# ltronchin/LatentAugment

Measured on AMD Instinct MI355X. Metric: augmented images/sec (256^2, 20 latent steps), higher is better.
Workload: dtype f32 (scaled split-fp16x2 on fp16 MFMA, fp32 accumulate); 1 GPU; SG2 config-f 256x256 2-ch, random-init G, batch=8/GPU, 20 latent steps; global_batch=8, parallelism=dp1

## Files before the change

### latentaugment_amd/csrc/la_conv_bf16.hip

```cpp
#include "la_conv_device.h"
#include <atomic>
#include <type_traits>

typedef __bf16 bf16x8 __attribute__((ext_vector_type(8)));
typedef _Float16 f16x8 __attribute__((ext_vector_type(8)));

#define FMT_BF16X3 3
#define FMT_BF16X2 2
#define FMT_F16X2 16
#define PRESPLIT_HDR 512

template <bool F16>
__device__ __forceinline__ f32x16 la_mma(bf16x8 a, bf16x8 b, f32x16 c) {
    if constexpr (F16) return __builtin_amdgcn_mfma_f32_32x32x16_f16(__builtin_bit_cast(f16x8, a), __builtin_bit_cast(f16x8, b), c, 0, 0, 0);
    else return __builtin_amdgcn_mfma_f32_32x32x16_bf16(a, b, c, 0, 0, 0);
}

#define KCB 32

__host__ __device__ static inline int pack_mp(int M) { return (M + 31) & ~31; }
__device__ __forceinline__ long pack_slab_offset(int m, int k) {
    return ((((long)(m >> 5) * 2 + (k >> 4)) * 64 + ((k >> 3) & 1) * 32 + (m & 31)) << 3) + (k & 7);
}
__global__ void la_pack_bf16_kernel(const float* __restrict__ w, __bf16* __restrict__ out, int cout, int cin, int ktaps,
// ... 241 lines not shown
__global__ __launch_bounds__(256) void la_presplit_t_kernel(const float* __restrict__ in, long in_bstride,
                                                           const float* __restrict__ scale, int scale_stride,
                                                           const float* __restrict__ xscale, int xs_fan, unsigned* __restrict__ out, int C, long HW,
                                                           LaInMask mk) {
    constexpr int EW = F16 ? 1 : 2;
    __shared__ unsigned tile[EW][64][33];
    const int cc = blockIdx.y, b = blockIdx.z, nck = gridDim.y;
    const long p0 = (long)blockIdx.x * 64;
    if (mk.p_hi > 0 && (p0 + 64 <= mk.p_lo || p0 >= mk.p_hi)) return;
    const float xs = F16 ? la_xs_get(xscale, b, xs_fan) : 1.f;
    {
        const int px = threadIdx.x & 63, cg = threadIdx.x >> 6;
        const long p = p0 + px;
#pragma unroll
        for (int i = 0; i < 8; ++i) {
            const int cl = cg * 8 + i, c = cc * KCB + cl;
            float v = 0.f;
            if (c < C && p < HW) {
                const long o = (long)b * in_bstride + (long)c * HW + p;
                v = in[o] * ((scale ? scale[(long)b * scale_stride + c] : 1.f) * xs);
                if (mk.y) v *= la_act_bwd_from_y(mk.y[o], mk.act, mk.alpha, mk.gain, mk.clamp);
                v *= mk.in_gain;
            }
            if (F16) {
                const _Float16 h = (_Float16)v;
                const _Float16 l = (_Float16)(v - (float)h);
                tile[0][px][cl] = (unsigned)__builtin_bit_cast(unsigned short, h) | ((unsigned)__builtin_bit_cast(unsigned short, l) << 16);
            } else {
                unsigned short t[3];
#pragma unroll
                for (int q = 0; q < 3; ++q) {
                    const __bf16 h = (__bf16)v;
                    t[q] = __builtin_bit_cast(unsigned short, h);
                    v -= (float)h;
                }
                tile[0][px][cl] = (unsigned)t[0] | ((unsigned)t[1] << 16);
                tile[EW - 1][px][cl] = (unsigned)t[2];
            }
        }
    }
    __syncthreads();
    {
        const int px = threadIdx.x >> 2, qt = threadIdx.x & 3;
        const long p = p0 + px;
        if (p < HW) {
            unsigned* op = out + (((long)b * nck + cc) * HW + p) * (KCB * EW) + qt * 8 * EW;
            if (F16) {
                unsigned e[8];
#pragma unroll
                for (int k = 0; k < 8; ++k) e[k] = tile[0][px][qt * 8 + k];
                uint4* rec = reinterpret_cast<uint4*>(out + (((long)b * nck + cc) * HW + p) * KCB);
                rec[qt] = make_uint4(__builtin_amdgcn_perm(e[1], e[0], 0x05040100u), __builtin_amdgcn_perm(e[3], e[2], 0x05040100u),
                                     __builtin_amdgcn_perm(e[5], e[4], 0x05040100u), __builtin_amdgcn_perm(e[7], e[6], 0x05040100u));
                rec[4 + qt] = make_uint4(__builtin_amdgcn_perm(e[1], e[0], 0x07060302u), __builtin_amdgcn_perm(e[3], e[2], 0x07060302u),
                                         __builtin_amdgcn_perm(e[5], e[4], 0x07060302u), __builtin_amdgcn_perm(e[7], e[6], 0x07060302u));
            } else {
#pragma unroll
                for (int k = 0; k < 4; ++k)
                    reinterpret_cast<uint4*>(op)[k] = make_uint4(tile[0][px][qt * 8 + 2 * k], tile[EW - 1][px][qt * 8 + 2 * k],
                                                                 tile[0][px][qt * 8 + 2 * k + 1], tile[EW - 1][px][qt * 8 + 2 * k + 1]);
            }
        }
    }
}

static inline size_t presplit_hdr_bytes(int B, int C) { return (PRESPLIT_HDR + (size_t)B * C * PM_NS * 4 + 255) & ~(size_t)255; }
size_t la_conv_presplit_bytes(int B, int C, int Hin, int Win) {
    return (size_t)B * la_cdiv(C, KCB) * KCB * Hin * Win * 8 + 16 + presplit_hdr_bytes(B, C);
}

static int prepare_scale(LaConvArgs& a, hipStream_t stream) {
    if (a.precision != LA_PREC_F16X2 || a.acc_scale_x) return LA_OK;
    const long HW = (long)a.Hin * a.Win;
    const size_t hb = presplit_hdr_bytes(a.B, a.C);
    LA_CHECK_ARG(a.ws && a.ws_bytes >= hb, "conv: split precisions need a workspace (la_modconv_workspace_bytes)");
    LA_CHECK_ARG(((size_t)a.ws & 15) == 0, "conv: workspace must be 16-byte aligned");
    LA_CHECK_ARG(a.B <= 64, "conv: split precisions support at most 64 samples per launch");
    char* base = static_cast<char*>(a.ws);
    float* xscale = reinterpret_cast<float*>(base);
    float* pm = reinterpret_cast<float*>(base + PRESPLIT_HDR);
    int ns = (int)(HW / 8192);
    ns = ns < 1 ? 1 : (ns > PM_NS ? PM_NS : ns);
    if (a.in_pmax) {
        hipLaunchKernelGGL(la_xscale_pmax_kernel, dim3(a.B), dim3(1024), 0, stream, a.in_pmax, a.in_pmax_nseg > 0 ? a.in_pmax_nseg : 1, a.in_scale,
                           a.scale_stride, xscale, a.C, 1.f);
    } else {
        hipLaunchKernelGGL(la_plane_absmax_kernel, dim3(ns, a.C, a.B), dim3(256), 0, stream, a.in, a.in_bstride, a.in_scale,
                           a.scale_stride, pm, a.C, HW, ns);
        hipLaunchKernelGGL(la_xscale_kernel, dim3(a.B), dim3(256), 0, stream, pm, xscale, a.C * ns);
    }
    LA_CHECK_LAUNCH();
    a.acc_scale_x = xscale; a.acc_scale_fan = 1;
    a.ws = base + hb;
    a.ws_bytes -= hb;
    return LA_OK;
}

bool la_conv_bf16_uses_halo(const LaConvArgs& a) {
    if (a.precision == LA_PREC_F32 || a.in_q) return false;
    if (a.in_mask_y || (a.in_gain != 0.f && a.in_gain != 1.f)) return false;
    if (a.in_sy != 1 || a.in_sx != 1 || a.out_sy != 1 || a.out_sx != 1 || a.out_oy != 0 || a.out_ox != 0) return false;
    if ((a.Gx & 31) != 0 || (a.Gy & 3) != 0 || a.Gy != a.Hout || a.Gx != a.Wout || a.ntaps != 9) return false;
    if ((long)a.Gy * a.Gx < (la_dev_knob(LA_KNOB_HALO_MING) ? la_dev_knob(LA_KNOB_HALO_MING) : 1157)) return false;
    if ((long)a.C * a.Hin * a.Win >= (1l << 28) || a.C > 4096) return false;
    for (int t = 0; t < a.ntaps; ++t)
        if (a.tap_dy[t] < -1 || a.tap_dy[t] > 1 || a.tap_dx[t] < -1 || a.tap_dx[t] > 1) return false;
    return true;
}

int la_conv_prepare_input(LaConvArgs& a, hipStream_t stream) {
    if (a.precision == LA_PREC_F32 || a.in_q) return LA_OK;
    const long HW = (long)a.Hin * a.Win;
    struct Bracket { int slot; hipStream_t st; ~Bracket() { la_prof_close(slot, st); } };
    if (la_conv_bf16_uses_halo(a)) {
        if (a.precision != LA_PREC_F16X2 || a.acc_scale_x) return LA_OK;
        Bracket br{la_prof_open(LA_PC_PRESPLIT, 0.0, a.in_pmax ? 0.0 : 4.0 * a.B * (double)a.C * HW * (a.in_bstride ? 1.0 : 1.0 / a.B), stream), stream};
        return prepare_scale(a, stream);
    }
    Bracket br{la_prof_open(LA_PC_PRESPLIT, 0.0, 4.0 * a.B * (double)a.C * HW * ((a.in_bstride ? 1.0 : 1.0 / a.B) + 1.0), stream), stream};
    const size_t qb = la_conv_presplit_bytes(a.B, a.C, a.Hin, a.Win);
    LA_CHECK_ARG(a.ws && a.ws_bytes >= qb, "conv: split precisions need a workspace (la_modconv_workspace_bytes)");
    LA_CHECK_ARG(((size_t)a.ws & 15) == 0, "conv: workspace must be 16-byte aligned");
    LA_CHECK_ARG(a.B <= 64, "conv: split precisions support at most 64 samples per launch");
    LA_CHECK_ARG(qb < 0x7ff00000u, "conv: pre-split operand too large for 32-bit buffer offsets");
    char* base = static_cast<char*>(a.ws);
    const size_t ws_bytes = a.ws_bytes;
    const dim3 pgrid((unsigned)la_cdiv(HW, 64), (unsigned)la_cdiv(a.C, KCB), (unsigned)a.B);
    const LaInMask mk{a.in_mask_y, a.in_mask_act, a.in_mask_alpha, a.in_mask_gain, a.in_mask_clamp, a.in_gain != 0.f ? a.in_gain : 1.f,
                      a.in_row_hi > 0 ? (long)a.in_row_lo * a.Win : 0, a.in_row_hi > 0 ? (long)a.in_row_hi * a.Win : 0};
    LA_CHECK_ARG((!a.in_mask_y && mk.in_gain == 1.f) || a.acc_scale_x || a.precision != LA_PREC_F16X2, "conv: an input mask needs a preset operand scale");
    if (a.precision == LA_PREC_F16X2) {
        int rc = prepare_scale(a, stream);
        if (rc) return rc;
        void* q = a.ws;
        hipLaunchKernelGGL(la_presplit_t_kernel<true>, pgrid, dim3(256), 0, stream, a.in, a.in_bstride, a.in_scale, a.scale_stride,
                           a.acc_scale_x, a.acc_scale_fan, (unsigned*)q, a.C, HW, mk);
        a.in_q = q;
    } else {
        void* q = base + presplit_hdr_bytes(a.B, a.C);
        hipLaunchKernelGGL(la_presplit_t_kernel<false>, pgrid, dim3(256), 0, stream, a.in, a.in_bstride, a.in_scale, a.scale_stride,
                           (const float*)nullptr, 0, (unsigned*)q, a.C, HW, mk);
        a.in_q = q;
    }
    LA_CHECK_LAUNCH();
    const size_t off = (qb + 255) & ~(size_t)255;
    a.ws = ws_bytes > off ? base + off : nullptr;
    a.ws_bytes = ws_bytes > off ? ws_bytes - off : 0;
    return LA_OK;
}

typedef unsigned int u32x4 __attribute__((ext_vector_type(4)));
typedef unsigned int u32x2 __attribute__((ext_vector_type(2)));
#define BPITCH 64
template <int MT, bool SPLIT, int FMT, int WV, int MF = 0>
__global__ __launch_bounds__(256) __attribute__((amdgpu_waves_per_eu(WV))) void la_conv_bf16_kernel(LaConvArgs a_in) {
    static_assert(MF == 0 ? WV == 2 : (MF <= 2 && WV == 3 && FMT == FMT_F16X2 && MT == 128),
                  "the 16x16x32 forms exist for the three-wave fp16 x2 kernel on 128-row tiles, the 32x32x16 form for two waves");
    LaConvArgs a = a_in;
    int bz = blockIdx.z;
    int bx = blockIdx.x;
    if (a_in.nphase > 0) {
        int ph;
        if (SPLIT) {
            ph = 0;
#pragma unroll
            for (int q = 1; q < LA_CONV_MAX_PHASES; ++q)
                if (q < a_in.nphase && bx >= a_in.ph[q].tile0) ph = q;
            bx -= a_in.ph[ph].tile0;
            a.splitk_ws = a_in.splitk_ws + a_in.ph[ph].ws_off;
        } else {
            ph = bz / a_in.B;
            bz -= ph * a_in.B;
        }
        a.Gy = a_in.ph[ph].Gy; a.Gx = a_in.ph[ph].Gx; a.out_oy = a_in.ph[ph].out_oy; a.out_ox = a_in.ph[ph].out_ox; a.ntaps = a_in.ph[ph].ntaps;
#pragma unroll
        for (int t = 0; t < LA_CONV_PHASE_TAPS; ++t) { a.tap_dy[t] = a_in.ph[ph].tap_dy[t]; a.tap_dx[t] = a_in.ph[ph].tap_dx[t]; a.tap_w[t] = a_in.ph[ph].tap_w[t]; }
    }
    constexpr int NTERM = FMT == FMT_BF16X3 ? 3 : 2;
    constexpr bool F16 = FMT == FMT_F16X2;
    constexpr int WM_ = MT == 128 ? 4 : 2;
    constexpr int WN_ = 4 / WM_;
    constexpr int TM = 1;
    constexpr int NJ = 4 / WN_;
    constexpr int EB = F16 ? 4 : 8;
    constexpr int BPLANE = NT * BPITCH;
    constexpr int BBUF = NTERM * BPLANE;
    extern __shared__ __attribute__((aligned(16))) unsigned char smem[];
    float (*red)[MT] = reinterpret_cast<float (*)[MT]>(smem);

    const int tid = threadIdx.x;
    const int lane = tid & 63, wid = tid >> 6;
    const int wm = wid / WN_, wn = wid % WN_;
    int ntile = bx;
    const int m0 = blockIdx.y * MT;
    const int G = a.Gy * a.Gx;
    const int Ntot = SPLIT ? a.B * G : G;
    if (!SPLIT) {
        int t0 = 0, nt = (int)gridDim.x;
        if (a.row_hi > 0) {
            const int tall = (G + NT - 1) / NT;
            t0 = (a.row_lo * a.Gx) / NT;
            int t1 = ((a.row_hi < a.Gy ? a.row_hi : a.Gy) * a.Gx + NT - 1) / NT;
            t1 = t1 < tall ? t1 : tall;
            nt = t1 - t0;
            for (int j = (int)blockIdx.x; j < tall - nt; j += (int)gridDim.x) la_conv_zero_partials<MT>(a, bz, m0, j < t0 ? j : j + nt);
            const int n8 = (int)gridDim.x;
            if ((n8 & 7) == 0) ntile = (blockIdx.x & 7) * (n8 >> 3) + (blockIdx.x >> 3);
            if (ntile >= nt) return;
        } else if ((nt & 7) == 0) ntile = (blockIdx.x & 7) * (nt >> 3) + (blockIdx.x >> 3);
        ntile += t0;
    }
    if (!SPLIT && (long)ntile * NT >= G) return;
    const int l31 = lane & 31, lh = lane >> 5;

    const int n_l = tid & (NT - 1);
    const int khalf = tid >> 7;
    const int nidx_l = ntile * NT + n_l;
    const bool nvalid = nidx_l < Ntot;
    const int b_l = SPLIT ? (nvalid ? nidx_l / G : 0) : bz;
    const int g_l = SPLIT ? nidx_l - b_l * G : nidx_l;
    const int gy_l = nvalid ? g_l / a.Gx : 0;
    const int gx_l = nvalid ? g_l - gy_l * a.Gx : 0;
    const int iy0 = gy_l * a.in_sy, ix0 = gx_l * a.in_sx;
    const unsigned HWin = (unsigned)(a.Hin * a.Win);
    const int vy0 = a.in_row_hi > 0 ? a.in_row_lo : 0, vy1 = a.in_row_hi > 0 ? a.in_row_hi : a.Hin;
    constexpr bool PIECES = FMT == FMT_F16X2;
    constexpr unsigned OOB = 0x7ff00000u;
    unsigned plin[4] = {0u, 0u, 0u, 0u}, pinv[4] = {0u, 0u, 0u, 0u};
    if constexpr (PIECES) {
#pragma unroll
        for (int k = 0; k < 4; ++k) {
            const int n_k = k * 32 + (tid >> 3);
            const int nidx = ntile * NT + n_k;
            const bool pv = nidx < Ntot;
            const int bb = SPLIT ? (pv ? nidx / G : 0) : bz;
            const int g = SPLIT ? nidx - bb * G : nidx;
            const int gy = pv ? g / a.Gx : 0, gx = pv ? g - gy * a.Gx : 0;
            const int py = gy * a.in_sy, px = gx * a.in_sx;
            const unsigned base = (SPLIT ? (unsigned)bb * ((unsigned)((a.C + KCB - 1) / KCB) * KCB * HWin * 4u) : 0u) + (unsigned)(tid & 7) * 16u;
            plin[k] = base + (unsigned)(py * a.Win + px) * (unsigned)(KCB * EB);
            unsigned m = 0u;
#pragma unroll
            for (int t = 0; t < LA_CONV_MAX_TAPS; ++t) {
                const int iy = py + a.tap_dy[t], ix = px + a.tap_dx[t];
                const bool bad = !pv || iy < vy0 || iy >= vy1 || ix < 0 || ix >= a.Win;
                m |= (bad ? 1u : 0u) << t;
            }
            pinv[k] = m;
        }
    }

    const int nck = (a.C + KCB - 1) / KCB;
    int ck_beg = 0, ck_end = nck;
    if (SPLIT) {
        const int per = (nck + a.ksplit - 1) / a.ksplit;
        ck_beg = blockIdx.z * per;
        ck_end = ck_beg + per < nck ? ck_beg + per : nck;
    }
    const int ntaps = a.ntaps;
    const int nstep = ck_end > ck_beg ? (ck_end - ck_beg) * ntaps : 0;
    const long term_elems = a.wgt_bf16_term_elems;
    const unsigned samp_bytes = (unsigned)nck * KCB * HWin * EB;
    const auto rs_in = __builtin_amdgcn_make_buffer_rsrc(
        const_cast<char*>(static_cast<const char*>(a.in_q)) + (SPLIT ? (size_t)0 : (size_t)bz * samp_bytes), 0,
        (int)(SPLIT ? samp_bytes * (unsigned)a.B : samp_bytes), 0x00020000);
    const auto rs_w = __builtin_amdgcn_make_buffer_rsrc(
        const_cast<char*>(static_cast<const char*>(a.wgt_bf16)) + (F16 ? pack_f16_offset(term_elems) : 0), 0, (int)(NTERM * term_elems * 2),
        0x00020000);
    const unsigned lane_base = (SPLIT ? (unsigned)b_l * samp_bytes : 0u) + (unsigned)(khalf * 16) * EB;

    unsigned long long dypack = 0ull, dxpack = 0ull, wpack = 0ull;
#pragma unroll
    for (int t = 0; t < LA_CONV_MAX_TAPS; ++t) {
        dypack |= (unsigned long long)((a.tap_dy[t] + 8) & 15) << (4 * t);
        dxpack |= (unsigned long long)((a.tap_dx[t] + 8) & 15) << (4 * t);
        wpack |= (unsigned long long)(a.tap_w[t] & 15) << (4 * t);
    }

    unsigned ex[16], ey[NTERM == 3 ? 16 : 1];
    bool ok_r = false;
    auto load_b = [&](int cc, int t) {
        if constexpr (PIECES) {
            const int dy = (int)((dypack >> (4 * t)) & 15u) - 8, dx = (int)((dxpack >> (4 * t)) & 15u) - 8;
            const unsigned delta = (unsigned)((dy * a.Win + dx) * (KCB * EB));
            const unsigned so = (unsigned)cc * HWin * (KCB * EB);
#pragma unroll
            for (int k = 0; k < 4; ++k) {
                const int bad = __builtin_amdgcn_sbfe((int)pinv[k], (unsigned)t, 1u);
                const u32x4 v = __builtin_amdgcn_raw_buffer_load_b128(rs_in, (plin[k] + delta) | ((unsigned)bad & OOB), so, 0);
                ex[4 * k] = v.x; ex[4 * k + 1] = v.y; ex[4 * k + 2] = v.z; ex[4 * k + 3] = v.w;
            }
            return;
        }
        const int iy = iy0 + (int)((dypack >> (4 * t)) & 15u) - 8, ix = ix0 + (int)((dxpack >> (4 * t)) & 15u) - 8;
        ok_r = nvalid && iy >= vy0 && iy < vy1 && ix >= 0 && ix < a.Win;
        const int iyc = iy < 0 ? 0 : (iy >= a.Hin ? a.Hin - 1 : iy), ixc = ix < 0 ? 0 : (ix >= a.Win ? a.Win - 1 : ix);
        const unsigned vo = lane_base + (unsigned)(iyc * a.Win + ixc) * (KCB * EB);
        const unsigned so = (unsigned)cc * HWin * (KCB * EB);
        if (NTERM == 3) {
#pragma unroll
            for (int k = 0; k < 8; ++k) {
                const u32x4 v = __builtin_amdgcn_raw_buffer_load_b128(rs_in, vo, so + 16 * k, 0);
                ex[2 * k] = v.x; ey[NTERM == 3 ? 2 * k : 0] = v.y; ex[2 * k + 1] = v.z; ey[NTERM == 3 ? 2 * k + 1 : 0] = v.w;
            }
        } else if (F16) {
#pragma unroll
            for (int k = 0; k < 4; ++k) {
                const u32x4 v = __builtin_amdgcn_raw_buffer_load_b128(rs_in, vo, so + 16 * k, 0);
                ex[4 * k] = v.x; ex[4 * k + 1] = v.y; ex[4 * k + 2] = v.z; ex[4 * k + 3] = v.w;
            }
        } else {
#pragma unroll
            for (int k = 0; k < 8; ++k) {
                const u32x4 v = __builtin_amdgcn_raw_buffer_load_b128(rs_in, vo, so + 16 * k, 0);
                ex[2 * k] = v.x; ex[2 * k + 1] = v.z;
            }
        }
    };
    const int wrow = n_l * BPITCH, wsw = (n_l >> 2) & 3;
    auto write_b = [&](unsigned char* buf) {
        if constexpr (PIECES) {
            const int wsw = MF ? ((tid >> 5) & 1) << 1 : (tid >> 5);
            unsigned char* p0 = buf + ((tid >> 2) & 1) * BPLANE + (tid >> 3) * BPITCH + ((((tid & 3) ^ wsw) & 3) << 4);
#pragma unroll
            for (int k = 0; k < 4; ++k)
                *reinterpret_cast<uint4*>(p0 + k * 32 * BPITCH) = make_uint4(ex[4 * k], ex[4 * k + 1], ex[4 * k + 2], ex[4 * k + 3]);
            return;
        }
#pragma unroll
        for (int q = 0; q < NTERM; ++q) {
            const unsigned sel = q == 1 ? 0x07060302u : 0x05040100u;
            unsigned w[8];
#pragma unroll
            for (int d = 0; d < 8; ++d) {
                const unsigned e0 = q == 2 ? ey[NTERM == 3 ? 2 * d : 0] : ex[2 * d];
                const unsigned e1 = q == 2 ? ey[NTERM == 3 ? 2 * d + 1 : 0] : ex[2 * d + 1];
                const unsigned v = __builtin_amdgcn_perm(e1, e0, sel);
                w[d] = ok_r ? v : 0u;
            }
            unsigned char* p = buf + q * BPLANE + wrow;
            *reinterpret_cast<uint4*>(p + ((((khalf * 2) ^ wsw) & 3) << 4)) = make_uint4(w[0], w[1], w[2], w[3]);
            *reinterpret_cast<uint4*>(p + ((((khalf * 2 + 1) ^ wsw) & 3) << 4)) = make_uint4(w[4], w[5], w[6], w[7]);
        }
    };
    const int rsw = (l31 >> 2) & 3;
    const int rbase = (wn * NJ * 32 + l31) * BPITCH;
    auto read_b = [&](const unsigned char* buf, int ks, bf16x8 (&dst)[NTERM][NJ]) {
        const int o = rbase + ((((ks * 2 + lh) ^ rsw) & 3) << 4);
#pragma unroll
        for (int j = 0; j < NJ; ++j)
#pragma unroll
            for (int q = 0; q < NTERM; ++q) dst[q][j] = *reinterpret_cast<const bf16x8*>(buf + q * BPLANE + j * 32 * BPITCH + o);
    };

    const int Mp = pack_mp(a.M);
    unsigned a_off[TM];
#pragma unroll
    for (int i = 0; i < TM; ++i) {
        int mblk = (m0 + wm * (MT / WM_) + i * 32) >> 5;
        mblk = mblk < (Mp >> 5) ? mblk : (Mp >> 5) - 1;
        a_off[i] = (unsigned)mblk * 2048u + (unsigned)lane * 16u;
    }
    const unsigned slab_bytes = (unsigned)Mp * KCB * 2u;
    const unsigned term_bytes = (unsigned)term_elems * 2u;
    auto load_a = [&](int cc, int t, int ks, bf16x8 (&dst)[NTERM][TM]) {
        const unsigned tw = (unsigned)((wpack >> (4 * t)) & 15u);
        const unsigned so = (tw * nck + cc) * slab_bytes + ks * 1024;
#pragma unroll
        for (int q = 0; q < NTERM; ++q)
#pragma unroll
            for (int i = 0; i < TM; ++i)
                dst[q][i] = __builtin_bit_cast(bf16x8, __builtin_amdgcn_raw_buffer_load_b128(rs_w, a_off[i], so + q * term_bytes, 0));
    };

    f32x16 acc[TM][NJ];
#pragma unroll
    for (int i = 0; i < TM; ++i)
#pragma unroll
        for (int j = 0; j < NJ; ++j)
#pragma unroll
            for (int r = 0; r < 16; ++r) acc[i][j][r] = 0.f;
    auto mma_step = [&](bf16x8 (&af)[NTERM][TM], bf16x8 (&bf)[NTERM][NJ]) {
#pragma unroll
        for (int i = 0; i < TM; ++i)
#pragma unroll
            for (int j = 0; j < NJ; ++j) {
                if constexpr (NTERM == 3) {
                    acc[i][j] = la_mma<F16>(af[2][i], bf[0][j], acc[i][j]);
                    acc[i][j] = la_mma<F16>(af[0][i], bf[2][j], acc[i][j]);
                    acc[i][j] = la_mma<F16>(af[1][i], bf[1][j], acc[i][j]);
                }
                acc[i][j] = la_mma<F16>(af[1][i], bf[0][j], acc[i][j]);
                acc[i][j] = la_mma<F16>(af[0][i], bf[1][j], acc[i][j]);
                acc[i][j] = la_mma<F16>(af[0][i], bf[0][j], acc[i][j]);
            }
    };

    if constexpr (MF >= 1) {
      typedef float f32x4 __attribute__((ext_vector_type(4)));
      const int c16 = lane & 15, kq = lane >> 4;
      f32x4 acc16[2][8];
#pragma unroll
      for (int mi = 0; mi < 2; ++mi)
#pragma unroll
          for (int n = 0; n < 8; ++n) acc16[mi][n] = f32x4{0.f, 0.f, 0.f, 0.f};
      if (nstep > 0) {
        int c1 = ck_beg, t1 = 0;
        auto adv = [&](int& c, int& t) {
            if (t + 1 < ntaps) ++t;
            else if (c + 1 < ck_end) { ++c; t = 0; }
        };
        int mblk16 = (m0 + wm * 32) >> 5;
        mblk16 = mblk16 < (Mp >> 5) ? mblk16 : (Mp >> 5) - 1;
        const unsigned a16_off = (unsigned)mblk16 * 2048u + (unsigned)(kq * 32 + c16) * 16u;
        auto load_a16 = [&](int cc, int t, int mi, f16x8 (&dst)[2]) {
            const unsigned tw = (unsigned)((wpack >> (4 * t)) & 15u);
            const unsigned so = (tw * nck + cc) * slab_bytes;
#pragma unroll
            for (int q = 0; q < 2; ++q)
                dst[q] = __builtin_bit_cast(f16x8, __builtin_amdgcn_raw_buffer_load_b128(rs_w, a16_off + (unsigned)mi * 256u, so + q * term_bytes, 0));
        };
        const int rb16 = c16 * BPITCH + (((kq ^ (((c16 >> 2) & 1) << 1)) & 3) << 4);
        auto read_b16 = [&](const unsigned char* buf, int n, f16x8 (&dst)[2]) {
#pragma unroll
            for (int q = 0; q < 2; ++q) dst[q] = *reinterpret_cast<const f16x8*>(buf + q * BPLANE + n * 16 * BPITCH + rb16);
        };
        f16x8 a16[2][2], b16[4][2];
        const int c0 = c1, t0 = t1;
      if constexpr (MF == 2) {
        load_b(c0, t0);
        adv(c1, t1);
        int c2 = c1, t2 = t1;
        write_b(smem);
        __builtin_amdgcn_sched_barrier(0);
        load_b(c1, t1);
        adv(c2, t2);
        write_b(smem + BBUF);
        __builtin_amdgcn_sched_barrier(0);
        load_b(c2, t2);
        __builtin_amdgcn_sched_barrier(0);
        load_a16(c0, t0, 0, a16[0]);
        __builtin_amdgcn_sched_barrier(0);
        load_a16(c0, t0, 1, a16[1]);
        __builtin_amdgcn_sched_barrier(0);
        __syncthreads();
        adv(c2, t2);
#pragma unroll
        for (int n = 0; n < 4; ++n) read_b16(smem, n, b16[n]);
        int ib = 0;
#pragma unroll 1
        for (int s = 0; s < nstep; ++s) {
            const int ib1 = ib == 2 ? 0 : ib + 1, ib2 = ib1 == 2 ? 0 : ib1 + 1;
            const unsigned char* cur = smem + ib * BBUF;
            const unsigned char* nx1 = smem + ib1 * BBUF;
            write_b(smem + ib2 * BBUF);
            load_b(c2, t2);
            __builtin_amdgcn_sched_barrier(0);
            const bool more = s + 1 < nstep;
#pragma unroll
            for (int q4 = 0; q4 < 4; ++q4) {
                const int hf = q4 >> 1, mi = q4 & 1;
#pragma unroll
                for (int k = 0; k < 4; ++k) {
                    const int n = hf * 4 + k;
                    f16x8 (&bs)[2] = b16[k];
                    acc16[mi][n] = __builtin_amdgcn_mfma_f32_16x16x32_f16(a16[mi][1], bs[0], acc16[mi][n], 0, 0, 0);
                    acc16[mi][n] = __builtin_amdgcn_mfma_f32_16x16x32_f16(a16[mi][0], bs[1], acc16[mi][n], 0, 0, 0);
                    acc16[mi][n] = __builtin_amdgcn_mfma_f32_16x16x32_f16(a16[mi][0], bs[0], acc16[mi][n], 0, 0, 0);
                    if (mi == 1) {
                        if (hf == 0) read_b16(cur, 4 + k, bs);
                        else if (more) read_b16(nx1, k, bs);
                    }
                    __builtin_amdgcn_sched_barrier(0);
                }
                if (q4 >= 2) load_a16(c1, t1, mi, a16[mi]);
            }
            adv(c1, t1);
            adv(c2, t2);
            ib = ib1;
            __syncthreads();
        }
      } else {
        load_b(c0, t0);
        adv(c1, t1);
        int c2 = c1, t2 = t1;
        write_b(smem);
        __builtin_amdgcn_sched_barrier(0);
        load_b(c1, t1);
        __builtin_amdgcn_sched_barrier(0);
        load_a16(c0, t0, 0, a16[0]);
        __builtin_amdgcn_sched_barrier(0);
        load_a16(c0, t0, 1, a16[1]);
        __builtin_amdgcn_sched_barrier(0);
        __syncthreads();
        adv(c2, t2);
#pragma unroll 1
        for (int s = 0; s < nstep; ++s) {
            const unsigned char* cur = smem + (s & 1) * BBUF;
            unsigned char* nxt = smem + ((s + 1) & 1) * BBUF;
#pragma unroll
            for (int n = 0; n < 4; ++n) read_b16(cur, n, b16[n]);
            write_b(nxt);
            load_b(c2, t2);
            __builtin_amdgcn_sched_barrier(0);
#pragma unroll
            for (int q4 = 0; q4 < 4; ++q4) {
                const int hf = q4 >> 1, mi = q4 & 1;
#pragma unroll
                for (int k = 0; k < 4; ++k) {
                    const int n = hf * 4 + k;
                    f16x8 (&bs)[2] = b16[k];
                    acc16[mi][n] = __builtin_amdgcn_mfma_f32_16x16x32_f16(a16[mi][1], bs[0], acc16[mi][n], 0, 0, 0);
                    acc16[mi][n] = __builtin_amdgcn_mfma_f32_16x16x32_f16(a16[mi][0], bs[1], acc16[mi][n], 0, 0, 0);
                    acc16[mi][n] = __builtin_amdgcn_mfma_f32_16x16x32_f16(a16[mi][0], bs[0], acc16[mi][n], 0, 0, 0);
                    if (mi == 1 && hf == 0) read_b16(cur, 4 + k, bs);
                    __builtin_amdgcn_sched_barrier(0);
                }
                if (q4 >= 2) load_a16(c1, t1, mi, a16[mi]);
            }
            c1 = c2; t1 = t2;
            adv(c2, t2);
            __syncthreads();
        }
      }
      }
      {
        float* tb = reinterpret_cast<float*>(smem) + wid * (64 * 36);
#pragma unroll
        for (int hf = 0; hf < 2; ++hf) {
            if (hf) __syncthreads();
#pragma unroll
            for (int mi = 0; mi < 2; ++mi)
#pragma unroll
                for (int n4 = 0; n4 < 4; ++n4) {
                    const int n = hf * 4 + n4;
                    *reinterpret_cast<f32x4*>(tb + (n4 * 16 + c16) * 36 + mi * 16 + kq * 4) = acc16[mi][n];
                }
            __syncthreads();
#pragma unroll
            for (int jj = 0; jj < 2; ++jj)
#pragma unroll
                for (int g = 0; g < 4; ++g) {
                    const f32x4 v = *reinterpret_cast<const f32x4*>(tb + (jj * 32 + l31) * 36 + 8 * g + 4 * lh);
#pragma unroll
                    for (int r = 0; r < 4; ++r) acc[0][hf * 2 + jj][4 * g + r] = v[r];
                }
        }
        __syncthreads();
      }
    } else
    if (nstep > 0) {
        int c1 = ck_beg, t1 = 0;
        auto adv = [&](int& c, int& t) {
            if (t + 1 < ntaps) ++t;
            else if (c + 1 < ck_end) { ++c; t = 0; }
        };
        bf16x8 acur[2][NTERM][TM], anxt[2][NTERM][TM], bf0[NTERM][NJ], bf1[NTERM][NJ];
        const int c0 = c1, t0 = t1;
        load_b(c0, t0);
        adv(c1, t1);
        int c2 = c1, t2 = t1;
        write_b(smem);
        __builtin_amdgcn_sched_barrier(0);
        load_b(c1, t1);
        __builtin_amdgcn_sched_barrier(0);
        load_a(c0, t0, 0, acur[0]);
        load_a(c0, t0, 1, acur[1]);
        __builtin_amdgcn_sched_barrier(0);
        __syncthreads();
        adv(c2, t2);
#pragma unroll 1
        for (int s = 0; s < nstep; ++s) {
            const unsigned char* cur = smem + (s & 1) * BBUF;
            unsigned char* nxt = smem + ((s + 1) & 1) * BBUF;
            read_b(cur, 0, bf0);
            read_b(cur, 1, bf1);
            write_b(nxt);
            load_b(c2, t2);
            load_a(c1, t1, 0, anxt[0]);
            load_a(c1, t1, 1, anxt[1]);
            __builtin_amdgcn_sched_barrier(0);
            mma_step(acur[0], bf0);
            mma_step(acur[1], bf1);
#pragma unroll
            for (int ks = 0; ks < 2; ++ks)
#pragma unroll
                for (int q = 0; q < NTERM; ++q)
#pragma unroll
                    for (int i = 0; i < TM; ++i) acur[ks][q][i] = anxt[ks][q][i];
            c1 = c2; t1 = t2;
            adv(c2, t2);
            __syncthreads();
        }
    }
    if (F16) {
        const float iw = 1.f / a.acc_scale_w[0];
#pragma unroll
        for (int j = 0; j < NJ; ++j) {
            int bb = bz;
            if (SPLIT) { const int nidx = ntile * NT + (wn * NJ + j) * 32 + l31; bb = nidx < Ntot ? nidx / G : 0; }
            const float inv = iw / la_xs_get(a.acc_scale_x, bb, a.acc_scale_fan);
#pragma unroll
            for (int i = 0; i < TM; ++i)
#pragma unroll
                for (int r = 0; r < 16; ++r) acc[i][j][r] *= inv;
        }
    }
    la_conv_epilogue<MT, SPLIT, false, WM_>(a, acc, red, ntile, m0, G, Ntot, SPLIT ? -1 : bz);
}

#define HALO_W 34
#define HALO_PX (6 * HALO_W)
#define HPITCH 64
#define H_UNITS (8 * HALO_PX)
#define H_UPT 182
#ifdef LA_DEV
__device__ unsigned long long la_dbg_buf[1 << 18];
#define LA_STAMP_DECL LaStamp stv; stv.on = a.dbg_stamp != 0; stv.last = 0ull; for (int i_ = 0; i_ < 12; ++i_) stv.seg[i_] = 0ull; if (stv.on) stv.last = __builtin_amdgcn_s_memtime();
#define LA_STAMP(i) do { if (stv.on) { const unsigned long long t_ = __builtin_amdgcn_s_memtime(); stv.seg[i] += t_ - stv.last; stv.last = t_; } } while (0)
#define LA_STAMP_ARG , -1, &stv
#define LA_STAMP_OUT do { if (stv.on && (threadIdx.x & 63) == 0) { const long wv_ = ((long)blockIdx.x + (long)gridDim.x * (blockIdx.y + (long)gridDim.y * blockIdx.z)) * 4 + (threadIdx.x >> 6); \
    if (wv_ * 16 + 16 <= (1 << 18)) { for (int i_ = 0; i_ < 12; ++i_) la_dbg_buf[wv_ * 16 + i_] = stv.seg[i_]; la_dbg_buf[wv_ * 16 + 12] = stv.last; \
    unsigned hw_, xcc_; asm volatile("s_getreg_b32 %0, hwreg(HW_REG_HW_ID)" : "=s"(hw_)); asm volatile("s_getreg_b32 %0, hwreg(HW_REG_XCC_ID)" : "=s"(xcc_)); \
    la_dbg_buf[wv_ * 16 + 13] = hw_; la_dbg_buf[wv_ * 16 + 14] = xcc_; } } } while (0)
extern "C" int la_dev_dbg_read(unsigned long long* dst, long n) {
    return hipMemcpyFromSymbol(dst, HIP_SYMBOL(la_dbg_buf), (size_t)n * sizeof(unsigned long long), 0, hipMemcpyDeviceToHost) == hipSuccess ? 0 : -1;
}
#else
#define LA_STAMP_DECL
#define LA_STAMP(i)
#define LA_STAMP_ARG
#define LA_STAMP_OUT
#endif
template <int MT, int FMT, int WV, int MF = 0>
__global__ __launch_bounds__(256) __attribute__((amdgpu_waves_per_eu(WV))) void la_conv_bf16_halo_kernel(LaConvArgs a) {
    constexpr bool SB = WV == 3;
    constexpr bool M16 = (MF & 1) != 0, PSL = (MF & 4) != 0;
    static_assert(MF == 0 ? FMT != FMT_F16X2 : (MF == 4 || MF == 21) && FMT == FMT_F16X2, "MF 0 for the bf16 formats, MF 4 / 21 for fp16 x2");
    static_assert(!M16 || (MF == 21 && WV == 3 && MT == 128), "the 16x16x32 form (M16) is MF 21: pixel-stationary loader, every pixel "
                                                              "fragment read once per tap, three waves, 128-row tiles");
    constexpr int NTERM = FMT == FMT_BF16X3 ? 3 : 2;
    constexpr bool F16 = FMT == FMT_F16X2;
    constexpr int WM_ = MT / 32;
    constexpr int WN_ = 4 / WM_;
    constexpr int TM = 1;
    constexpr int NJ = 4 / WN_;
    constexpr int EB = 4;
    constexpr int HPLANE = HALO_PX * HPITCH;
    constexpr int HBUF = NTERM * HPLANE;
    extern __shared__ __attribute__((aligned(16))) unsigned char smem[];
    float (*red)[MT] = reinterpret_cast<float (*)[MT]>(smem);
    float* scl = reinterpret_cast<float*>(smem + (a.C > KCB ? 2 : 1) * HBUF);

    const int tid = threadIdx.x;
    const int lane = tid & 63, wid = tid >> 6;
    const int wm = wid / WN_, wn = wid % WN_;
    const int tpr = a.Gx >> 5;
    int nt = (int)gridDim.x;
    int r0 = 0, c0 = 0, cw = tpr;
    int ntile = blockIdx.x;
    if (a.row_hi > 0) {
        const int r1 = ((a.row_hi < a.Gy ? a.row_hi : a.Gy) + 3) >> 2;
        r0 = a.row_lo >> 2;
        if (a.col_hi > 0) { c0 = a.col_lo >> 5; cw = (((a.col_hi < a.Gx ? a.col_hi : a.Gx) + 31) >> 5) - c0; }
        nt = (r1 - r0) * cw;
        const int tall = (a.Gy >> 2) * tpr, n_out = tall - nt;
        for (int j = (int)blockIdx.x; j < n_out; j += (int)gridDim.x) {
            int otile, k = j;
            const int per = tpr - cw;
            if (k < r0 * tpr) otile = k;
            else if ((k -= r0 * tpr) < (r1 - r0) * per) { const int rr = k / per, kk = k - rr * per; otile = (r0 + rr) * tpr + (kk < c0 ? kk : kk + cw); }
            else otile = r1 * tpr + (k - (r1 - r0) * per);
            la_conv_zero_partials<MT>(a, (int)blockIdx.z, (int)blockIdx.y * MT, otile);
        }
        const int n8 = (int)gridDim.x;
        if ((n8 & 7) == 0) {
            const int q = nt >> 3, r = nt & 7, rot = gridDim.z >= 8 ? 1 : (gridDim.z >= 4 ? 2 : (gridDim.z >= 2 ? 4 : 0));
            const int kv = (int)((blockIdx.x + blockIdx.z * rot) & 7), idx = (int)(blockIdx.x >> 3);
            if (idx >= q + (kv < r ? 1 : 0)) return;
            ntile = kv * q + (kv < r ? kv : r) + idx;
        } else if (ntile >= nt) return;
        const int rr = ntile / cw;
        ntile = (r0 + rr) * tpr + c0 + (ntile - rr * cw);
    } else if ((nt & 7) == 0) ntile = (blockIdx.x & 7) * (nt >> 3) + (blockIdx.x >> 3);
    const int m0 = blockIdx.y * MT;
    const int b = blockIdx.z;
    const int G = a.Gy * a.Gx;
    const int tyb = ntile / tpr, txb = ntile - tyb * tpr;
    const int y0 = tyb * 4 - 1, x0 = txb * 32 - 1;
    const unsigned HWin = (unsigned)(a.Hin * a.Win);
    const int vy0 = a.in_row_hi > 0 ? a.in_row_lo : 0, vy1 = a.in_row_hi > 0 ? a.in_row_hi : a.Hin;
    const int nck = (a.C + KCB - 1) / KCB;
    const long term_elems = a.wgt_bf16_term_elems;
    const int l31 = lane & 31, lh = lane >> 5;
    const auto rs_in = __builtin_amdgcn_make_buffer_rsrc(
        const_cast<float*>(a.in) + (size_t)b * a.in_bstride, 0, (int)((unsigned)a.C * HWin * EB), 0x00020000);
    const auto rs_w = __builtin_amdgcn_make_buffer_rsrc(
        const_cast<char*>(static_cast<const char*>(a.wgt_bf16)) + (F16 ? pack_f16_offset(term_elems) : 0), 0, (int)(NTERM * term_elems * 2),
        0x00020000);

    unsigned long long shpack = 0ull, wpack = 0ull;
    unsigned xpack = 0u;
#pragma unroll
    for (int t = 0; t < 9; ++t) {
        shpack |= (unsigned long long)((1 + a.tap_dy[t]) * HALO_W + (1 + a.tap_dx[t])) << (7 * t);
        wpack |= (unsigned long long)a.tap_w[t] << (4 * t);
        xpack |= (unsigned)(1 + a.tap_dx[t]) << (2 * t);
    }

    struct Slice { float x[4]; int wr, c0; bool ok; };
    auto slice_load = [&](int cc, int t, Slice& sl, bool live = true) {
        const int lt = (tid + 64 * t) & 255;
        int u = t * H_UPT + (lt < H_UPT ? lt : H_UPT - 1);
        const bool valid = live && lt < H_UPT && u < H_UNITS;
        u = u < H_UNITS ? u : H_UNITS - 1;
        const int c4 = u / HALO_PX, hp = u - c4 * HALO_PX;
        const int hy = hp / HALO_W, hx = hp - hy * HALO_W;
        const int iy = y0 + hy, ix = x0 + hx;
        sl.ok = iy >= vy0 && iy < vy1 && ix >= 0 && ix < a.Win;
        const int iyc = iy < 0 ? 0 : (iy >= a.Hin ? a.Hin - 1 : iy), ixc = ix < 0 ? 0 : (ix >= a.Win ? a.Win - 1 : ix);
        const unsigned off = (unsigned)(iyc * a.Win + ixc) * EB;
        const int swz = hp >> 2;
        sl.wr = valid ? hp * HPITCH + ((((c4 >> 1) ^ swz) & 3) << 4) + (c4 & 1) * 8 : -1;
        sl.c0 = cc * KCB + c4 * 4;
        const bool fast = cc * KCB + KCB <= a.C;
#pragma unroll
        for (int j = 0; j < 4; ++j) {
            unsigned vo, so;
            if (fast) { vo = live ? (unsigned)(c4 * 4) * HWin * EB + off : 0u; so = live ? (unsigned)(cc * KCB + j) * HWin * EB : 0u; }
            else {
                const int c = cc * KCB + c4 * 4 + j;
                vo = (unsigned)(c < a.C ? c : a.C - 1) * HWin * EB + off;
                so = 0u;
            }
            sl.x[j] = __builtin_bit_cast(float, __builtin_amdgcn_raw_buffer_load_b32(rs_in, vo, so, 0));
        }
    };
    auto slice_write = [&](unsigned char* buf, const Slice& sl) {
        if (sl.wr >= 0) {
            typedef float f32x2 __attribute__((ext_vector_type(2)));
            typedef __bf16 bf16x2_t __attribute__((ext_vector_type(2)));
            const float4 f = *reinterpret_cast<const float4*>(scl + sl.c0);
            float p[4] = {sl.x[0] * f.x, sl.x[1] * f.y, sl.x[2] * f.z, sl.x[3] * f.w};
#pragma unroll
            for (int q = 0; q < NTERM; ++q) {
                const bf16x2_t h0 = __builtin_convertvector(f32x2{p[0], p[1]}, bf16x2_t), h1 = __builtin_convertvector(f32x2{p[2], p[3]}, bf16x2_t);
// ... 256 lines not shown
            if constexpr (NTERM == 3) {
                acc[0][j] = la_mma<F16>(af[2][0], bf[0][j], acc[0][j]);
                acc[0][j] = la_mma<F16>(af[0][0], bf[2][j], acc[0][j]);
                acc[0][j] = la_mma<F16>(af[1][0], bf[1][j], acc[0][j]);
            }
            acc[0][j] = la_mma<F16>(af[1][0], bf[0][j], acc[0][j]);
            acc[0][j] = la_mma<F16>(af[0][0], bf[1][j], acc[0][j]);
            acc[0][j] = la_mma<F16>(af[0][0], bf[0][j], acc[0][j]);
            if (refill) {
                int o;
                if constexpr (PSL) o = (lb ^ (ks << 5)) + (wn * NJ + j) * HALO_W * HPITCH;
                else {
                    const int p = (wn * NJ + j) * HALO_W + shift + l31;
                    o = p * HPITCH + ((((ks * 2 + lh) ^ (p >> 2)) & 3) << 4);
                }
#pragma unroll
                for (int q = 0; q < NTERM; ++q) bf[q][j] = *reinterpret_cast<const bf16x8*>(buf + q * HPLANE + o);
            }
            __builtin_amdgcn_sched_barrier(0);
        }
    };
    for (int cc = 0; cc < nck; ++cc) {
        const unsigned char* cur = smem + (cc & 1) * HBUF;
        unsigned char* nxt = smem + ((cc + 1) & 1) * HBUF;
        const bool has_next = cc + 1 < nck;
        Slice sl;
        sl.wr = -1;
        sl.ok = false;
        float psx[4] = {0.f, 0.f, 0.f, 0.f};
        int lb = PSL ? lane_b((int)(shpack & 127u), (int)(xpack & 3u)) : 0;
        read_b(cur, (int)(shpack & 127u), 0, bf, lb);
#pragma unroll 1
        for (int t = 0; t < 9; ++t) {
            const int shift = (int)((shpack >> (7 * t)) & 127u);
            const int tn = t + 1 < 9 ? t + 1 : 0;
            const int ccn = t + 1 < 9 ? cc : (has_next ? cc + 1 : 0);
            const int shift_n = (int)((shpack >> (7 * (t + 1 < 9 ? t + 1 : 8))) & 127u);
            float4 psf = make_float4(0.f, 0.f, 0.f, 0.f);
            if constexpr (PSL) { if (has_next && t >= 1) psf = ps_factors(cc + 1, t - 1); }
            mma_refill(acur[0], cur, shift, 1, true, lb);
            if constexpr (PSL) lb = lane_b(shift_n, (int)((xpack >> (2 * (t + 1 < 9 ? t + 1 : 8))) & 3u));
            load_a(ccn, tn, 0, acur[0]);
            if constexpr (PSL) {
                if (has_next && t >= 1) ps_write(nxt, t - 1, psx, psf);
                ps_load(has_next ? cc + 1 : cc, t, psx);
            } else {
                slice_write(nxt, sl);
                slice_load(has_next ? cc + 1 : cc, t, sl, has_next);
            }
            __builtin_amdgcn_sched_barrier(0);
            mma_refill(acur[1], cur, shift_n, 0, t + 1 < 9, lb);
            load_a(ccn, tn, 1, acur[1]);
        }
        if constexpr (!PSL) slice_write(nxt, sl);
        __syncthreads();
    }
  } else {
    bf16x8 bf0[NTERM][NJ], bf1[NTERM][NJ];
    auto chunk = [&](int cc, auto has_next) {
        constexpr bool NEXT = decltype(has_next)::value;
        const unsigned char* cur = smem + (cc & 1) * HBUF;
        unsigned char* nxt = smem + ((cc + 1) & 1) * HBUF;
        Slice sl;
        sl.wr = -1;
        sl.ok = false;
        float psx[4] = {0.f, 0.f, 0.f, 0.f};
        int lb = PSL ? lane_b((int)(shpack & 127u), (int)(xpack & 3u)) : 0;
        read_b(cur, (int)(shpack & 127u), 0, bf0, lb);
#pragma unroll 1
        for (int t = 0; t < 9; ++t) {
            const int shift = (int)((shpack >> (7 * t)) & 127u);
            const int tn = t + 1 < 9 ? t + 1 : 0;
            const int ccn = t + 1 < 9 ? cc : (NEXT ? cc + 1 : 0);
            const int shift_n = (int)((shpack >> (7 * (t + 1 < 9 ? t + 1 : 8))) & 127u);
            float4 psf = make_float4(0.f, 0.f, 0.f, 0.f);
            if constexpr (PSL) { if (NEXT && t >= 1) psf = ps_factors(cc + 1, t - 1); }
            read_b(cur, shift, 1, bf1, lb);
            mma_step(acur[0], bf0);
            __builtin_amdgcn_sched_barrier(0);
            load_a(ccn, tn, 0, acur[0]);
            if constexpr (PSL) lb = lane_b(shift_n, (int)((xpack >> (2 * (t + 1 < 9 ? t + 1 : 8))) & 3u));
            read_b(cur, shift_n, 0, bf0, lb);
            if (NEXT) {
                if constexpr (PSL) {
                    if (t >= 1) ps_write(nxt, t - 1, psx, psf);
                    ps_load(cc + 1, t, psx);
                } else {
                    slice_write(nxt, sl);
                    slice_load(cc + 1, t, sl);
                }
            }
            mma_step(acur[1], bf1);
            __builtin_amdgcn_sched_barrier(0);
            load_a(ccn, tn, 1, acur[1]);
        }
        if (NEXT && !PSL) slice_write(nxt, sl);
    };
    for (int cc = 0; cc < nck; ++cc) {
        if (cc + 1 < nck) chunk(cc, std::true_type{});
        else chunk(cc, std::false_type{});
        __syncthreads();
    }
  }
    if (F16) {
        const float inv = 1.f / (a.acc_scale_w[0] * la_xs_get(a.acc_scale_x, b, a.acc_scale_fan));
#pragma unroll
        for (int i = 0; i < TM; ++i)
#pragma unroll
            for (int j = 0; j < NJ; ++j)
#pragma unroll
                for (int r = 0; r < 16; ++r) acc[i][j][r] *= inv;
    }
    la_conv_epilogue<MT, false, true, WM_>(a, acc, red, ntile, m0, G, G);
}

#ifdef LA_DEV
#define HALO_LDS_CAP (160 * 1024)
#else
#define HALO_LDS_CAP (2 * 3 * HALO_PX * HPITCH + 4096 * (int)sizeof(float))
#endif
template <int MT, int FMT, int WV, int MF>
static int launch_halo(const LaConvArgs& as, dim3 grid, size_t lds, hipStream_t stream) {
    static std::atomic<bool> cap_set[64];
    int dev = 0;
    if (hipGetDevice(&dev) != hipSuccess || dev < 0 || dev >= 64) dev = 0;
    if (!cap_set[dev].load(std::memory_order_acquire)) {
        const hipError_t e = hipFuncSetAttribute(reinterpret_cast<const void*>(&la_conv_bf16_halo_kernel<MT, FMT, WV, MF>),
                                                 hipFuncAttributeMaxDynamicSharedMemorySize, HALO_LDS_CAP);
        if (e != hipSuccess) { la_set_error(hipGetErrorString(e)); return LA_ERR_HIP; }
        cap_set[dev].store(true, std::memory_order_release);
    }
    hipLaunchKernelGGL((la_conv_bf16_halo_kernel<MT, FMT, WV, MF>), grid, dim3(256), lds, stream, as);
    return LA_OK;
}

template <int FMT>
static int launch_bf16(const LaConvArgs& as, int MTsel, dim3 grid, bool split, hipStream_t stream) {
    constexpr int NTERM = FMT == FMT_BF16X3 ? 3 : 2;
    if (!split && la_conv_bf16_uses_halo(as)) {
        size_t lds = (size_t)(as.C > KCB ? 2 : 1) * NTERM * HALO_PX * HPITCH + (size_t)la_cdiv(as.C, KCB) * KCB * sizeof(float);
        const size_t epi = (size_t)160 * MTsel + (size_t)2048 * (MTsel / 32);
        if (lds < epi) lds = epi;
        if constexpr (FMT == FMT_F16X2) {
            if (MTsel == 128 && as.C > KCB) return launch_halo<128, FMT, 3, 21>(as, grid, lds + (size_t)la_dev_knob(LA_KNOB_HALO_LDSPAD) * 1024, stream);
            if (MTsel == 128) return launch_halo<128, FMT, 3, 4>(as, grid, lds, stream);
            if (MTsel == 64) return launch_halo<64, FMT, 2, 4>(as, grid, lds, stream);
            return launch_halo<32, FMT, 2, 4>(as, grid, lds, stream);
        } else {
            if (MTsel == 128) return launch_halo<128, FMT, NTERM == 2 ? 3 : 2, 0>(as, grid, lds, stream);
            if (MTsel == 64) return launch_halo<64, FMT, 2, 0>(as, grid, lds, stream);
            return launch_halo<32, FMT, 2, 0>(as, grid, lds, stream);
        }
    }
    const size_t lds = (size_t)2 * NTERM * NT * BPITCH;
    if (MTsel == 128) {
        if constexpr (FMT == FMT_F16X2) {
            const size_t lds_mf = lds > (size_t)4 * 64 * 36 * 4 ? lds : (size_t)4 * 64 * 36 * 4;
            if (split) hipLaunchKernelGGL((la_conv_bf16_kernel<128, true, FMT, 3, 1>), grid, dim3(256), lds_mf, stream, as);
            else hipLaunchKernelGGL((la_conv_bf16_kernel<128, false, FMT, 3, 2>), grid, dim3(256), (size_t)3 * NTERM * NT * BPITCH, stream, as);
        } else {
            if (split) hipLaunchKernelGGL((la_conv_bf16_kernel<128, true, FMT, 2>), grid, dim3(256), lds, stream, as);
            else hipLaunchKernelGGL((la_conv_bf16_kernel<128, false, FMT, 2>), grid, dim3(256), lds, stream, as);
        }
    } else {
        if (split) hipLaunchKernelGGL((la_conv_bf16_kernel<64, true, FMT, 2>), grid, dim3(256), lds, stream, as);
        else hipLaunchKernelGGL((la_conv_bf16_kernel<64, false, FMT, 2>), grid, dim3(256), lds, stream, as);
    }
    return LA_OK;
}

int la_conv_bf16_dispatch(const LaConvArgs& args, int MTsel, dim3 grid, bool split, hipStream_t stream) {
    LaConvArgs as = args;
    if (as.precision == LA_PREC_F16X2)
        as.acc_scale_w = reinterpret_cast<const float*>(static_cast<const char*>(as.wgt_bf16) + pack_wscale_offset(as.wgt_bf16_term_elems));
    if (as.precision == LA_PREC_BF16X3) return launch_bf16<FMT_BF16X3>(as, MTsel, grid, split, stream);
    if (as.precision == LA_PREC_F16X2) return launch_bf16<FMT_F16X2>(as, MTsel, grid, split, stream);
    return launch_bf16<FMT_BF16X2>(as, MTsel, grid, split, stream);
}
```

Measured before the change: 87.45 images/s.

## Stream fp16x2 activation tiles straight to LDS via buffer_load_lds triple-buffer ring

Replaces the register-staged global-to-LDS copy of activation pieces in the fp16x2 conv kernels with direct buffer-load-to-LDS DMA into a three-slot ring. A custom barrier waits on partial vmcnt so loads for later steps stay in flight. It also drops the MF=2 variant and the two-buffer MF=1 loop, and uses the ring for the 32x32 two-wave path, with LDS sized for three buffers. The aim is to cut VGPR pressure and ds_write instructions and to overlap loads more deeply, at the cost of larger LDS footprint and fragile hand-tuned waitcnt counts.

```diff
diff --git a/latentaugment_amd/csrc/la_conv_bf16.hip b/latentaugment_amd/csrc/la_conv_bf16.hip
--- a/latentaugment_amd/csrc/la_conv_bf16.hip
+++ b/latentaugment_amd/csrc/la_conv_bf16.hip
@@ -417,10 +417,17 @@
 typedef unsigned int u32x4 __attribute__((ext_vector_type(4)));
 typedef unsigned int u32x2 __attribute__((ext_vector_type(2)));
 #define BPITCH 64
+template <int N>
+__device__ __forceinline__ void la_ring_barrier() {
+    __builtin_amdgcn_sched_barrier(0);
+    asm volatile("s_waitcnt vmcnt(%0) lgkmcnt(0)" ::"n"(N) : "memory");
+    __builtin_amdgcn_s_barrier();
+    __builtin_amdgcn_sched_barrier(0);
+}
 template <int MT, bool SPLIT, int FMT, int WV, int MF = 0>
 __global__ __launch_bounds__(256) __attribute__((amdgpu_waves_per_eu(WV))) void la_conv_bf16_kernel(LaConvArgs a_in) {
-    static_assert(MF == 0 ? WV == 2 : (MF <= 2 && WV == 3 && FMT == FMT_F16X2 && MT == 128),
-                  "the 16x16x32 forms exist for the three-wave fp16 x2 kernel on 128-row tiles, the 32x32x16 form for two waves");
+    static_assert(MF == 0 ? WV == 2 : (MF == 1 && WV == 3 && FMT == FMT_F16X2 && MT == 128),
+                  "the 16x16x32 form exists for the three-wave fp16 x2 kernel on 128-row tiles, the 32x32x16 form for two waves");
     LaConvArgs a = a_in;
     int bz = blockIdx.z;
     int bx = blockIdx.x;
@@ -491,18 +498,21 @@
     const int vy0 = a.in_row_hi > 0 ? a.in_row_lo : 0, vy1 = a.in_row_hi > 0 ? a.in_row_hi : a.Hin;
     constexpr bool PIECES = FMT == FMT_F16X2;
     constexpr unsigned OOB = 0x7ff00000u;
-    unsigned plin[4] = {0u, 0u, 0u, 0u}, pinv[4] = {0u, 0u, 0u, 0u};
+    int wv_u = 0;
+    unsigned plin[2] = {0u, 0u}, pinv[2] = {0u, 0u};
     if constexpr (PIECES) {
-#pragma unroll
-        for (int k = 0; k < 4; ++k) {
-            const int n_k = k * 32 + (tid >> 3);
+        wv_u = __builtin_amdgcn_readfirstlane(wid);
+#pragma unroll
+        for (int k = 0; k < 2; ++k) {
+            const int n_k = (wid * 2 + k) * 16 + (lane >> 2);
             const int nidx = ntile * NT + n_k;
             const bool pv = nidx < Ntot;
             const int bb = SPLIT ? (pv ? nidx / G : 0) : bz;
             const int g = SPLIT ? nidx - bb * G : nidx;
             const int gy = pv ? g / a.Gx : 0, gx = pv ? g - gy * a.Gx : 0;
             const int py = gy * a.in_sy, px = gx * a.in_sx;
-            const unsigned base = (SPLIT ? (unsigned)bb * ((unsigned)((a.C + KCB - 1) / KCB) * KCB * HWin * 4u) : 0u) + (unsigned)(tid & 7) * 16u;
+            const int swz = MF ? ((n_k >> 2) & 1) << 1 : (n_k >> 2) & 3;
+            const unsigned base = (SPLIT ? (unsigned)bb * ((unsigned)((a.C + KCB - 1) / KCB) * KCB * HWin * 4u) : 0u) + (unsigned)((lane & 3) ^ swz) * 16u;
             plin[k] = base + (unsigned)(py * a.Win + px) * (unsigned)(KCB * EB);
             unsigned m = 0u;
 #pragma unroll
@@ -542,21 +552,24 @@
         wpack |= (unsigned long long)(a.tap_w[t] & 15) << (4 * t);
     }
 
-    unsigned ex[16], ey[NTERM == 3 ? 16 : 1];
-    bool ok_r = false;
-    auto load_b = [&](int cc, int t) {
+    auto dma_b = [&](unsigned char* buf, int cc, int t) {
         if constexpr (PIECES) {
             const int dy = (int)((dypack >> (4 * t)) & 15u) - 8, dx = (int)((dxpack >> (4 * t)) & 15u) - 8;
             const unsigned delta = (unsigned)((dy * a.Win + dx) * (KCB * EB));
             const unsigned so = (unsigned)cc * HWin * (KCB * EB);
 #pragma unroll
-            for (int k = 0; k < 4; ++k) {
+            for (int k = 0; k < 2; ++k) {
                 const int bad = __builtin_amdgcn_sbfe((int)pinv[k], (unsigned)t, 1u);
-                const u32x4 v = __builtin_amdgcn_raw_buffer_load_b128(rs_in, (plin[k] + delta) | ((unsigned)bad & OOB), so, 0);
-                ex[4 * k] = v.x; ex[4 * k + 1] = v.y; ex[4 * k + 2] = v.z; ex[4 * k + 3] = v.w;
-            }
-            return;
-        }
+                const unsigned vo = (plin[k] + delta) | ((unsigned)bad & OOB);
+                unsigned char* dst = buf + (wv_u * 2 + k) * 16 * BPITCH;
+                __builtin_amdgcn_raw_ptr_buffer_load_lds(rs_in, (__attribute__((address_space(3))) void*)dst, 16, vo, so, 0, 0);
+                __builtin_amdgcn_raw_ptr_buffer_load_lds(rs_in, (__attribute__((address_space(3))) void*)(dst + BPLANE), 16, vo, so + 64u, 0, 0);
+            }
+        }
+    };
+    unsigned ex[16], ey[NTERM == 3 ? 16 : 1];
+    bool ok_r = false;
+    auto load_b = [&](int cc, int t) {
         const int iy = iy0 + (int)((dypack >> (4 * t)) & 15u) - 8, ix = ix0 + (int)((dxpack >> (4 * t)) & 15u) - 8;
         ok_r = nvalid && iy >= vy0 && iy < vy1 && ix >= 0 && ix < a.Win;
         const int iyc = iy < 0 ? 0 : (iy >= a.Hin ? a.Hin - 1 : iy), ixc = ix < 0 ? 0 : (ix >= a.Win ? a.Win - 1 : ix);
@@ -568,12 +581,6 @@
                 const u32x4 v = __builtin_amdgcn_raw_buffer_load_b128(rs_in, vo, so + 16 * k, 0);
                 ex[2 * k] = v.x; ey[NTERM == 3 ? 2 * k : 0] = v.y; ex[2 * k + 1] = v.z; ey[NTERM == 3 ? 2 * k + 1 : 0] = v.w;
             }
-        } else if (F16) {
-#pragma unroll
-            for (int k = 0; k < 4; ++k) {
-                const u32x4 v = __builtin_amdgcn_raw_buffer_load_b128(rs_in, vo, so + 16 * k, 0);
-                ex[4 * k] = v.x; ex[4 * k + 1] = v.y; ex[4 * k + 2] = v.z; ex[4 * k + 3] = v.w;
-            }
         } else {
 #pragma unroll
             for (int k = 0; k < 8; ++k) {
@@ -584,14 +591,6 @@
     };
     const int wrow = n_l * BPITCH, wsw = (n_l >> 2) & 3;
     auto write_b = [&](unsigned char* buf) {
-        if constexpr (PIECES) {
-            const int wsw = MF ? ((tid >> 5) & 1) << 1 : (tid >> 5);
-            unsigned char* p0 = buf + ((tid >> 2) & 1) * BPLANE + (tid >> 3) * BPITCH + ((((tid & 3) ^ wsw) & 3) << 4);
-#pragma unroll
-            for (int k = 0; k < 4; ++k)
-                *reinterpret_cast<uint4*>(p0 + k * 32 * BPITCH) = make_uint4(ex[4 * k], ex[4 * k + 1], ex[4 * k + 2], ex[4 * k + 3]);
-            return;
-        }
 #pragma unroll
         for (int q = 0; q < NTERM; ++q) {
             const unsigned sel = q == 1 ? 0x07060302u : 0x05040100u;
@@ -692,24 +691,17 @@
         };
         f16x8 a16[2][2], b16[4][2];
         const int c0 = c1, t0 = t1;
-      if constexpr (MF == 2) {
-        load_b(c0, t0);
+        dma_b(smem, c0, t0);
         adv(c1, t1);
         int c2 = c1, t2 = t1;
-        write_b(smem);
         __builtin_amdgcn_sched_barrier(0);
-        load_b(c1, t1);
+        dma_b(smem + BBUF, c1, t1);
         adv(c2, t2);
-        write_b(smem + BBUF);
-        __builtin_amdgcn_sched_barrier(0);
-        load_b(c2, t2);
         __builtin_amdgcn_sched_barrier(0);
         load_a16(c0, t0, 0, a16[0]);
         __builtin_amdgcn_sched_barrier(0);
         load_a16(c0, t0, 1, a16[1]);
-        __builtin_amdgcn_sched_barrier(0);
-        __syncthreads();
-        adv(c2, t2);
+        la_ring_barrier<4>();
 #pragma unroll
         for (int n = 0; n < 4; ++n) read_b16(smem, n, b16[n]);
         int ib = 0;
@@ -718,8 +710,7 @@
             const int ib1 = ib == 2 ? 0 : ib + 1, ib2 = ib1 == 2 ? 0 : ib1 + 1;
             const unsigned char* cur = smem + ib * BBUF;
             const unsigned char* nx1 = smem + ib1 * BBUF;
-            write_b(smem + ib2 * BBUF);
-            load_b(c2, t2);
+            dma_b(smem + ib2 * BBUF, c2, t2);
             __builtin_amdgcn_sched_barrier(0);
             const bool more = s + 1 < nstep;
 #pragma unroll
@@ -743,51 +734,8 @@
             adv(c1, t1);
             adv(c2, t2);
             ib = ib1;
-            __syncthreads();
-        }
-      } else {
-        load_b(c0, t0);
-        adv(c1, t1);
-        int c2 = c1, t2 = t1;
-        write_b(smem);
-        __builtin_amdgcn_sched_barrier(0);
-        load_b(c1, t1);
-        __builtin_amdgcn_sched_barrier(0);
-        load_a16(c0, t0, 0, a16[0]);
-        __builtin_amdgcn_sched_barrier(0);
-        load_a16(c0, t0, 1, a16[1]);
-        __builtin_amdgcn_sched_barrier(0);
-        __syncthreads();
-        adv(c2, t2);
-#pragma unroll 1
-        for (int s = 0; s < nstep; ++s) {
-            const unsigned char* cur = smem + (s & 1) * BBUF;
-            unsigned char* nxt = smem + ((s + 1) & 1) * BBUF;
-#pragma unroll
-            for (int n = 0; n < 4; ++n) read_b16(cur, n, b16[n]);
-            write_b(nxt);
-            load_b(c2, t2);
-            __builtin_amdgcn_sched_barrier(0);
-#pragma unroll
-            for (int q4 = 0; q4 < 4; ++q4) {
-                const int hf = q4 >> 1, mi = q4 & 1;
-#pragma unroll
-                for (int k = 0; k < 4; ++k) {
-                    const int n = hf * 4 + k;
-                    f16x8 (&bs)[2] = b16[k];
-                    acc16[mi][n] = __builtin_amdgcn_mfma_f32_16x16x32_f16(a16[mi][1], bs[0], acc16[mi][n], 0, 0, 0);
-                    acc16[mi][n] = __builtin_amdgcn_mfma_f32_16x16x32_f16(a16[mi][0], bs[1], acc16[mi][n], 0, 0, 0);
-                    acc16[mi][n] = __builtin_amdgcn_mfma_f32_16x16x32_f16(a16[mi][0], bs[0], acc16[mi][n], 0, 0, 0);
-                    if (mi == 1 && hf == 0) read_b16(cur, 4 + k, bs);
-                    __builtin_amdgcn_sched_barrier(0);
-                }
-                if (q4 >= 2) load_a16(c1, t1, mi, a16[mi]);
-            }
-            c1 = c2; t1 = t2;
-            adv(c2, t2);
-            __syncthreads();
-        }
-      }
+            la_ring_barrier<4>();
+        }
       }
       {
         float* tb = reinterpret_cast<float*>(smem) + wid * (64 * 36);
@@ -822,6 +770,46 @@
         };
         bf16x8 acur[2][NTERM][TM], anxt[2][NTERM][TM], bf0[NTERM][NJ], bf1[NTERM][NJ];
         const int c0 = c1, t0 = t1;
+      if constexpr (PIECES) {
+        static_assert(!PIECES || NTERM * TM == 2, "the ring's counts assume four weight loads per step");
+        dma_b(smem, c0, t0);
+        adv(c1, t1);
+        int c2 = c1, t2 = t1;
+        __builtin_amdgcn_sched_barrier(0);
+        load_a(c0, t0, 0, acur[0]);
+        load_a(c0, t0, 1, acur[1]);
+        __builtin_amdgcn_sched_barrier(0);
+        dma_b(smem + BBUF, c1, t1);
+        adv(c2, t2);
+        la_ring_barrier<4>();
+        int ib = 0;
+#pragma unroll 1
+        for (int s = 0; s < nstep; ++s) {
+            const int ib1 = ib == 2 ? 0 : ib + 1, ib2 = ib1 == 2 ? 0 : ib1 + 1;
+            const unsigned char* cur = smem + ib * BBUF;
+            read_b(cur, 0, bf0);
+            read_b(cur, 1, bf1);
+            load_a(c1, t1, 0, anxt[0]);
+            load_a(c1, t1, 1, anxt[1]);
+            __builtin_amdgcn_sched_barrier(0);
+            dma_b(smem + ib2 * BBUF, c2, t2);
+            __builtin_amdgcn_sched_barrier(0);
+            mma_step(acur[0], bf0);
+            mma_step(acur[1], bf1);
+#pragma unroll
+            for (int ks = 0; ks < 2; ++ks)
+#pragma unroll
+                for (int q = 0; q < NTERM; ++q)
+#pragma unroll
+                    for (int i = 0; i < TM; ++i) acur[ks][q][i] = anxt[ks][q][i];
+            c1 = c2; t1 = t2;
+            adv(c2, t2);
+            ib = ib1;
+            la_ring_barrier<4>();
+        }
+        asm volatile("s_waitcnt vmcnt(0)" ::: "memory");
+        __builtin_amdgcn_s_barrier();
+      } else {
         load_b(c0, t0);
         adv(c1, t1);
         int c2 = c1, t2 = t1;
@@ -857,6 +845,7 @@
             adv(c2, t2);
             __syncthreads();
         }
+      }
     }
     if (F16) {
         const float iw = 1.f / a.acc_scale_w[0];
@@ -1419,12 +1408,11 @@
             return launch_halo<32, FMT, 2, 0>(as, grid, lds, stream);
         }
     }
-    const size_t lds = (size_t)2 * NTERM * NT * BPITCH;
+    const size_t lds = (size_t)(FMT == FMT_F16X2 ? 3 : 2) * NTERM * NT * BPITCH;
     if (MTsel == 128) {
         if constexpr (FMT == FMT_F16X2) {
-            const size_t lds_mf = lds > (size_t)4 * 64 * 36 * 4 ? lds : (size_t)4 * 64 * 36 * 4;
-            if (split) hipLaunchKernelGGL((la_conv_bf16_kernel<128, true, FMT, 3, 1>), grid, dim3(256), lds_mf, stream, as);
-            else hipLaunchKernelGGL((la_conv_bf16_kernel<128, false, FMT, 3, 2>), grid, dim3(256), (size_t)3 * NTERM * NT * BPITCH, stream, as);
+            if (split) hipLaunchKernelGGL((la_conv_bf16_kernel<128, true, FMT, 3, 1>), grid, dim3(256), lds, stream, as);
+            else hipLaunchKernelGGL((la_conv_bf16_kernel<128, false, FMT, 3, 1>), grid, dim3(256), lds, stream, as);
         } else {
             if (split) hipLaunchKernelGGL((la_conv_bf16_kernel<128, true, FMT, 2>), grid, dim3(256), lds, stream, as);
             else hipLaunchKernelGGL((la_conv_bf16_kernel<128, false, FMT, 2>), grid, dim3(256), lds, stream, as);
```

Result: no change. 87.81 images/s (median of 6 runs) (+0.4%).
